# bcgsc/goldrush

Measured on AMD Instinct MI355X. Metric: reads/s through GoldRush-Path (hash + miBF query), higher is better.
Workload: dtype u64

## Files before the change

goldrush_amd/csrc/grp_kernels.inc:

```

__device__ inline uint64_t
window_lo(const uint32_t* sBases, uint32_t b)
{
  uint32_t bit = b * 2u;
  uint32_t wi = bit >> 5;
  uint32_t sh = bit & 31u;
  uint64_t lo = (uint64_t)sBases[wi] | ((uint64_t)sBases[wi + 1] << 32);
  uint64_t w = lo >> sh;
  if (sh) {
    w |= (uint64_t)sBases[wi + 2] << (64u - sh);
  }
  return w;
}

struct Win
{
  uint64_t lo;
  const uint32_t* src;
  uint32_t b;
};

__device__ inline Win
window_at(const uint32_t* sBases, uint32_t b)
{
// ... 749 lines not shown
      }
    }
    if (k == rank + 1) {
      stc(&f.ovf_ids[slot], id);
      return;
    }
    slot = (slot + 1) & f.ovf_mask;
  }
}

struct InsertTable
{
  unsigned long long* keys;
  unsigned long long* masks;
  unsigned long long* locs;
  uint32_t* slots;
  uint32_t* counter;
  uint64_t cap_mask;
};


struct DevStreamCtl
{
  uint32_t first = 0;
  uint32_t* tiles_done = nullptr;
  uint32_t* abort = nullptr;
  const uint32_t* abort_host = nullptr;
  grp_read_decision* dec = nullptr;
  uint32_t* next_tile = nullptr;
  uint32_t* park = nullptr;
  uint32_t n_tiles = 0;
  uint32_t early_park = 1;
  unsigned long long* executed = nullptr;
  grp_decide_params dp{};
  uint32_t* g_ids = nullptr;
  uint8_t* g_asg = nullptr;
  uint64_t* g_scratch = nullptr;
  uint32_t* ctl = nullptr;
  const uint32_t* cmd_host = nullptr;
  uint32_t* ack_host = nullptr;
  uint32_t n_reads = 0;
  uint32_t n_decidable = 0;
  uint32_t cmd_while_busy = 0;
  InsertTable tb{};
  unsigned long long timeout_ticks = 0;
  uint32_t* tile_ver = nullptr;
  uint32_t* fp_tab[2] = { nullptr, nullptr };
  uint32_t fp_mask = 0;
  uint32_t* rel = nullptr;
  uint32_t* dbg = nullptr;
  uint32_t n_fp = 0;
  uint32_t fp_off = 0;
  uint32_t fp_words = 0;
};

constexpr uint32_t STREAM_TILE_HELD = 0xFFFFFFFEu;
constexpr uint32_t STREAM_TILE_BUSY = 0xFFFFFFFDu;
constexpr uint32_t STREAM_REDO_NONE = 0xFFFFFFFFu;
constexpr uint32_t STREAM_FULL_RESET = 0x80000000u;

__device__ inline uint32_t
slot_fp(uint64_t b, uint32_t off)
{
  const uint32_t x = ((uint32_t)b ^ ((uint32_t)(b >> 32) * 0x85EBCA6Bu)) * 0x9E3779B1u + off;
  return x ? x : 1u;
}

constexpr unsigned long long IR_LOC_MASK = (1ull << 58) - 1ull;

__device__ inline uint32_t
fp_home(uint32_t fp, uint32_t mask)
{
  return (fp ^ (fp >> 15)) & mask;
}

__device__ inline void
fp_put(uint32_t* tab, uint32_t mask, uint32_t fp)
{
  uint32_t slot = fp_home(fp, mask);
  for (;;) {
    uint32_t cur = ldc(&tab[slot]);
    if (cur == 0u) {
      cur = atomicCAS(&tab[slot], 0u, fp);
      if (cur == 0u) {
        return;
      }
    }
    if (cur == fp) {
      return;
    }
    slot = (slot + 1u) & mask;
  }
}

__device__ inline bool
fp_has(const uint32_t* tab, uint32_t mask, uint32_t fp)
{
  uint32_t slot = fp_home(fp, mask);
  for (;;) {
    const uint32_t cur = tab[slot];
    if (cur == 0u) {
      return false;
    }
    if (cur == fp) {
      return true;
    }
// ... 1102 lines not shown
  uint32_t idx[H];
#pragma unroll
  for (int s = 0; s < H; ++s) {
    have[s] = look[s] && grp_claim_epoch(k[s]) == bv.epoch;
    idx[s] = grp_claim_record(k[s]);
  }
  uint32_t chain[H];
  unsigned long long rk[H], ro[H];
#pragma unroll
  for (int s = 0; s < H; ++s) {
    chain[s] = have[s] ? bv.rec_chain[idx[s]] : BATCH_NONE;
    rk[s] = have[s] ? bv.rec_key[idx[s]] : 0ull;
    ro[s] = have[s] ? bv.rec_old[idx[s]] : 0ull;
  }
#pragma unroll
  for (int s = 0; s < H; ++s) {
    if (have[s]) {
      if (chain[s] == BATCH_NONE) {
        const uint32_t j = (uint32_t)(rk[s] & ((1ull << 26) - 1ull)) >> 8;
        const uint32_t writer = bv.ins[(size_t)j * 6] - bv.first;
        d[s] = (writer >= reader && (ro[s] >> 63)) ? (uint32_t)ro[s] : d[s];
      } else {
        d[s] = batch_view_log(bv, rank[s] + 1, reader, d[s]);
      }
    }
  }
}

__device__ inline uint32_t
batch_view_log(const DevBatchView& bv, unsigned long long key, uint32_t reader, uint32_t cur)
{
  uint64_t slot = (key * 0x9E3779B97F4A7C15ULL) >> 18 & bv.log_mask;
  for (;;) {
    const unsigned long long k = bv.log_keys[slot];
    if (k == key) {
      break;
    }
    if (k == 0) {
      return cur;
    }
    slot = (slot + 1) & bv.log_mask;
  }
  uint32_t best_w = BATCH_NONE, best_old = cur;
  for (uint32_t e = bv.log_head[slot]; e != BATCH_NONE; e = bv.log_next[e]) {
    const uint32_t w = bv.log_writer[e];
    if (w >= reader && w <= best_w) {
      best_w = w;
      best_old = bv.log_old[e];
    }
  }
  return best_old;
}

template<int H, int FR, int WT, bool ST, bool VER = false, bool GT = false>
__global__ void __launch_bounds__(THREADS, (ST && H <= 3) ? 3 : ((!ST && H >= 4 && H <= 5) ? 3 : 1))
k_query(DevFilter f,
        DevReads rd,
        const DevSeeds* __restrict__ sd,
        uint32_t tile_len,
        uint64_t tile_begin,
        const uint32_t* __restrict__ tile_idx,
        uint32_t hist_cap,
        uint32_t distinct_limit,
        grp_tile_summary* __restrict__ tiles_out,
        grp_id_count* __restrict__ lists_out,
        uint64_t lists_cap,
        unsigned long long* __restrict__ ctr,
        uint32_t* __restrict__ flagged_out,
        uint32_t flagged_cap,
        uint32_t direct_stride,
        uint32_t blk0,
        DevStreamCtl sc,
        DevBatchView bv,
        uint32_t* __restrict__ gtab = nullptr)
{
  if constexpr (VER && !ST) {
    if (bv.redo_count != nullptr && blockIdx.x >= *bv.redo_count) {
      return;
    }
  }
  extern __shared__ uint4 smem4[];
  ulonglong2* sTab = reinterpret_cast<ulonglong2*>(smem4);
  const uint32_t hn = frame_seeds<H>(sd);
  uint32_t* sKeys;
  uint32_t* sCnts;
  uint32_t* sBases;
  if constexpr (GT) {
    sKeys = gtab + (size_t)blockIdx.x * (hist_cap + hist_cap / 2u);
    sCnts = sKeys + hist_cap;
    sBases = reinterpret_cast<uint32_t*>(sTab + hn * sd->wmax * 4u);
  } else {
    sKeys = reinterpret_cast<uint32_t*>(sTab + hn * sd->wmax * 4u);
    sCnts = sKeys + hist_cap;
    sBases = sCnts + hist_cap / 2u;
  }
  auto tab_word = [&](const uint32_t* p) -> uint32_t {
    if constexpr (GT) {
      return __hip_atomic_load(p, __ATOMIC_RELAXED, __HIP_MEMORY_SCOPE_AGENT);
    } else {
      return *p;
    }
  };
  __shared__ uint32_t sListN, sDistinct, sOverflow, sListOff, sListW;
  __shared__ uint32_t sRed[2 * (THREADS / 64)];
  __shared__ uint32_t sBest[2 * (THREADS / 64)];
  __shared__ uint32_t sTile;
  __shared__ unsigned long long sDirectWord;
  __shared__ uint32_t sInsWave[THREADS / 64 + 1];
  __shared__ uint32_t sEv, sAct;
  __shared__ uint32_t sHeldTile[2], sHeldPasses[2];
  __shared__ uint32_t sBuf;
  __shared__ uint32_t sCut;
  __shared__ uint32_t sOwnRedo[2], sOwnRedoN;
  __shared__ uint32_t sWalkEnd;
  __shared__ uint32_t sGen;

  load_tab(sTab, sd);
  uint32_t nxt = 0;
  uint32_t stop = 0;
  uint32_t my_ev = 0;
  uint32_t phase = 0;
  bool host_abort_seen = false;
  uint32_t ev_next = 0;
  uint32_t pending_event = 0;
  uint32_t* const sFp = (ST && sc.ctl && sc.n_fp) ? reinterpret_cast<uint32_t*>(reinterpret_cast<char*>(smem4) + sc.fp_off) : nullptr;
  if constexpr (ST) {
    if (threadIdx.x == 0) {
      sHeldTile[0] = sHeldTile[1] = STREAM_REDO_NONE;
      sHeldPasses[0] = sHeldPasses[1] = 0u;
      sBuf = 0u;
      sCut = 0u;
      sOwnRedoN = 0u;
      sWalkEnd = 0u;
      sGen = 1u;
      if (sc.dbg) {
        stc(&sc.dbg[blockIdx.x], 0x00000001u);
        stc(&sc.dbg[4095], gridDim.x);
        stc(&sc.dbg[4096 + (blockIdx.x & 1023u)], (uint32_t)wall_clock64());
        stc(&sc.dbg[5120 + (blockIdx.x & 1023u)], (__builtin_amdgcn_s_getreg((16 - 1) << 11 | 4) & 0xFFFFu) | (__builtin_amdgcn_s_getreg((4 - 1) << 11 | 20) << 16));
      }
      if (__hip_atomic_load(sc.abort_host, __ATOMIC_RELAXED, __HIP_MEMORY_SCOPE_SYSTEM)) {
        atomicMin(sc.park, 0u);
        atomicMax(sc.next_tile, STREAM_STOP);
        __hip_atomic_store(sc.abort, 1u, __ATOMIC_RELAXED, __HIP_MEMORY_SCOPE_AGENT);
        stop = 1u;
        host_abort_seen = true;
      }
      if (sc.ctl) {
        uint32_t ph0 = 0;
        if (!stream_register(sc, &my_ev, &ph0)) {
          stop = 1u;
          host_abort_seen = true;
        }
        sEv = ph0;
        sGen = ldc(sc.ctl + SCT_GEN);
        sWalkEnd = ldc(sc.ctl + SCT_SCAN_END) & ~STREAM_FULL_RESET;
        ev_next = my_ev;
      }
      nxt = atomicAdd(sc.next_tile, 1u);
    }
    if (sc.ctl) {
      __syncthreads();
      phase = sEv;
    }
  }
  for (;;) {
  uint32_t out_idx;
  if constexpr (ST) {
    if (__builtin_expect(pending_event != 0u, 0)) {
      pending_event = 0u;
      if (threadIdx.x == 0 && sc.dbg) {
        stc(&sc.dbg[blockIdx.x], 0x10000000u | (my_ev & 0xFFFFu));
        stc(&sc.dbg[1024 + (blockIdx.x & 1023u)], (uint32_t)wall_clock64());
      }
      if (threadIdx.x == 0) {
        sAct = host_abort_seen ? STREAM_ACT_EXIT : stream_idle(sc, &my_ev);
        sEv = my_ev;
        ev_next = my_ev;
      }
      __syncthreads();
      if (sAct == STREAM_ACT_EXIT) {
        return;
      }
      if (sAct == STREAM_ACT_INSERT) {
        if (sFp != nullptr && threadIdx.x < 2u) {
          const uint32_t th = sHeldTile[threadIdx.x];
          if (th != STREAM_REDO_NONE) {
            stc(&sc.tile_ver[th], STREAM_TILE_HELD);
          }
        }
        if (threadIdx.x == 0 && sc.dbg) {
          stc(&sc.dbg[blockIdx.x], 0x20000000u | (my_ev & 0xFFFFu));
        }
        StreamInsertDone done;
        if (!stream_apply_insert<H, WT>(f, rd, sd, sTab, sBases, sInsWave, &sAct, tile_len, sc, sEv, phase, ctr, lists_cap, tile_idx, done)) {
          return;
        }
        const bool keep_none = (done.scan_end & STREAM_FULL_RESET) != 0u;
        if (threadIdx.x == 0) {
          sWalkEnd = done.scan_end & ~STREAM_FULL_RESET;
          sGen = done.gen;
        }
        if (done.rank == 0u && threadIdx.x == 0) {
          atomicAdd(sc.executed + (keep_none ? EXE_INSERTS_KEPT_NONE : EXE_INSERTS_KEPT), 1ull);
        }
        {
          const uint32_t* const changed = sc.fp_tab[done.par];
          for (uint32_t hb = 0; hb < 2u; ++hb) {
            __syncthreads();
            const uint32_t th = sHeldTile[hb];
            if (sFp == nullptr || th == STREAM_REDO_NONE) {
              continue;
            }
            const uint32_t rh = rd.tile_read[tile_begin + th];
            const uint32_t rjh = rh - sc.first;
            if (rjh < done.resume_read) {
              __syncthreads();
              if (threadIdx.x == 0) {
                sHeldTile[hb] = STREAM_REDO_NONE;
              }
              continue;
            }
            bool dirty = keep_none;
            const uint32_t nfp = keep_none ? 0u : sHeldPasses[hb] * (uint32_t)THREADS * (uint32_t)H;
#pragma unroll 4
            for (uint32_t q = threadIdx.x; q < nfp; q += THREADS) {
              const uint32_t fp = sFp[hb * sc.fp_words + q];
              const bool hit = fp != 0u && fp_has(changed, sc.fp_mask, fp);
              dirty = dirty | hit;
            }
            const bool any_dirty = __syncthreads_or(dirty ? 1 : 0) != 0;
// ... 14 lines not shown
              sTile = (atomicAdd(&sc.tiles_done[rjh], 1u) + 1u == nt_h) ? 1u : 0u;
            }
            __syncthreads();
            if (sTile != 0u && threadIdx.x < 64u) {
              stream_decide(sc, rjh, rd.tile0[rh] - tile_begin, nt_h, tiles_out, lists_out, lists_cap, reinterpret_cast<uint32_t*>(sKeys), min(STREAM_LDS_TILES, hist_cap * 6u / 40u));
            }
          }
          __syncthreads();
          if (threadIdx.x == 0) {
            nxt = atomicAdd(sc.next_tile, 1u);
          }
          if (threadIdx.x == 0) {
            stop = 0u;
          }
        }
      }
      __syncthreads();
    }
    if (threadIdx.x == 0) {
      uint32_t pick = STREAM_STOP;
      bool from_dispenser = false;
      if (sc.ctl && ev_next != my_ev) {
      } else {
        if (sc.ctl && sOwnRedoN != 0u) {
          pick = sOwnRedo[--sOwnRedoN];
        }
        while (pick == STREAM_STOP && nxt < sc.n_tiles) {
          const uint32_t cand = tile_idx ? tile_idx[nxt] : nxt;
          if (sc.ctl && nxt < sWalkEnd) {
            const uint32_t v = ldc(&sc.tile_ver[cand]);
            if (v == STREAM_TILE_HELD || v == STREAM_TILE_BUSY || (v != 0u && v == sGen)) {
              nxt = atomicAdd(sc.next_tile, 1u);
              continue;
            }
            if (v != 0u) {
              atomicAdd(sc.executed + EXE_REDONE_LOST, 1ull);
            }
          }
          pick = cand;
          from_dispenser = true;
        }
        if (stop && from_dispenser) {
          const uint32_t rj = rd.tile_read[tile_begin + pick] - sc.first;
          if (rj >= __hip_atomic_load(sc.park, __ATOMIC_RELAXED, __HIP_MEMORY_SCOPE_AGENT)) {
            pick = STREAM_STOP;
            from_dispenser = false;
          }
        }
      }
      sTile = pick;
      if (from_dispenser) {
        nxt = atomicAdd(sc.next_tile, 1u);
      }
      if (pick != STREAM_STOP && sc.ctl != nullptr && blockIdx.x < 32u) {
        stream_relay(sc);
      } else if (pick != STREAM_STOP && blockIdx.x < 32u) {
        if (__hip_atomic_load(sc.abort_host, __ATOMIC_RELAXED, __HIP_MEMORY_SCOPE_SYSTEM)) {
          atomicMin(sc.park, 0u);
          atomicMax(sc.next_tile, STREAM_STOP);
          __hip_atomic_store(sc.abort, 1u, __ATOMIC_RELAXED, __HIP_MEMORY_SCOPE_AGENT);
        }
      }
    }
    if (threadIdx.x == 0 && sc.dbg) {
      stc(&sc.dbg[blockIdx.x], 0x30000000u | (sTile & 0x0FFFFFFFu));
    }
    __syncthreads();
    out_idx = sTile;
    if (out_idx == STREAM_STOP) {
      if (!sc.ctl) {
        return;
      }
      pending_event = 1u;
      continue;
    }
  } else {
    out_idx = tile_idx ? tile_idx[blockIdx.x] : blockIdx.x + blk0;
  }
  const uint64_t t = tile_begin + out_idx;
  const uint32_t r = rd.tile_read[t];
  const uint32_t ti = (uint32_t)(t - rd.tile0[r]);
  if constexpr (VER && !ST) {
    if (bv.skip_read_ins != nullptr && r - bv.first < bv.skip_reads) {
      const uint32_t ji = bv.skip_read_ins[r - bv.first];
      if (ji != 0xFFFFFFFFu && ti >= bv.ins[(size_t)ji * 6 + 1] && ti < bv.ins[(size_t)ji * 6 + 2]) {
        return;
      }
    }
  }
  const uint32_t len = rd.len[r];
  const gr::geom::TileExtent ext = tile_extent(sd, tile_len, len, ti);
  const uint32_t start = ext.start, Lp = ext.Lp, frames = ext.frames;

  const uint32_t boff = stage_bases(sBases, rd.packed, rd.word_off[r], len, start, Lp);
  for (uint32_t i = threadIdx.x; i < hist_cap; i += THREADS) {
    sKeys[i] = 0u;
    if (i < hist_cap / 2u) {
      sCnts[i] = 0u;
    }
  }
  if (threadIdx.x == 0) {
    sListN = 0;
    sListW = 0;
    sDistinct = 0;
    sOverflow = 0;
    if constexpr (ST) {
      sCut = 0u;
      if (sFp != nullptr) {
        if (sc.n_fp > 1u) {
          sBuf ^= 1u;
        }
        sHeldTile[sBuf] = STREAM_REDO_NONE;
      }
    }
  }
  __syncthreads();
  if constexpr (ST) {
    if (threadIdx.x == 0) {
      atomicAdd(sc.executed + EXE_PROBES, (unsigned long long)frames * hn);
    }
  }
  uint32_t* const fp_cur = (ST && sFp != nullptr) ? sFp + sBuf * sc.fp_words : nullptr;

  uint32_t n_hit = 0, n_miss = 0;
  uint32_t last[H];
#pragma unroll
  for (int s = 0; s < H; ++s) {
    last[s] = Lp - sd->span[s];
  }
  const QuadLane ql = quad_lane();
  constexpr bool ROT = quad_rotated<H, FR, WT, ST, VER, GT>();
  const uint32_t pbytes = quad_piece_bytes(ql.sub);

  const uint32_t n_left = (H >= 2 && H <= GRP_H_GROUP && WT != GRP_WT_LONG) ? sd->n_left : 0u;
  constexpr uint32_t OV = (uint32_t)H - 1u, USE = 64u - OV;
  static_assert(THREADS == 256, "the helper-lane layout below is written for four waves per workgroup (my_wave == 3 is the last one, FBH = 3 * USE + 64)");
  constexpr uint32_t FBH = gr::geom::helper_pass_frames(H);
  const uint32_t ftile = frames_per_tile(sd, tile_len);
  const bool helper = n_left != 0u && (ftile + FBH * FR - 1u) / (FBH * FR) == (ftile + THREADS * FR - 1u) / (THREADS * FR);
  const uint32_t FB = helper ? FBH : (uint32_t)THREADS;
  const uint32_t my_wave = threadIdx.x >> 6, my_lane = threadIdx.x & 63u;
  const uint32_t my_off = helper ? (my_wave * USE + my_lane) : threadIdx.x;
  const bool my_real = helper ? (my_wave == 3u || my_lane < USE) : true;
  const bool my_tail_wave = helper ? my_wave == 3u : true;
  const uint32_t passes = (frames + FB * FR - 1u) / (FB * FR);
  uint64_t bk[FR][H];
  uint32_t off[FR][H];
  bool live_j[FR];
  auto positions = [&](uint32_t pp, uint64_t (&bk_)[FR][H], uint32_t (&off_)[FR][H], bool (&lv)[FR]) {
  if (n_left != 0u) {
#pragma unroll
    for (int j = 0; j < FR; ++j) {
      const uint32_t fr_raw = (pp * FR + j) * FB + my_off;
      const uint32_t fr = min(fr_raw, frames - 1u);
      lv[j] = my_real && fr_raw < frames;
      uint64_t hL, hRL, hR, hRR;
      seed_halves<WT, true, true>(sTab, sd, n_left, window_at(sBases, boff + fr), hL, hRL, hR, hRR);
      const uint64_t hv0 = (hL ^ hR) + (hRL ^ hRR);
#pragma unroll
      for (int s = 0; s < H; ++s) {
        uint64_t hv = hv0;
        if (s != 0) {
          uint64_t nR = __shfl_down((unsigned long long)hR, (unsigned)s, 64);
          uint64_t nRR = __shfl_down((unsigned long long)hRR, (unsigned)s, 64);
          if (my_tail_wave && my_lane + (uint32_t)s >= 64u) {
            uint64_t a, b;
            seed_halves<WT, false, true>(sTab, sd, n_left, window_at(sBases, boff + min(fr_raw + (uint32_t)s, frames - 1u)), a, b, nR, nRR);
          }
          if (lv[j]) {
            if (fr <= last[s]) {
              hv = (srol_small(hL, (uint32_t)s) ^ nR) + (hRL ^ srol_small(nRR, (uint32_t)s));
            } else {
              hv = seed_hash_t<WT>(sTab, sd, s, window_at(sBases, boff + last[s]));
            }
          }
        }
        const Probe p = grp_locate(f, hv);
        bk_[j][s] = p.b;
        off_[j][s] = p.off;
        if constexpr (ST) {
          if (fp_cur != nullptr) {
            fp_cur[((pp * FR + (uint32_t)j) * (uint32_t)THREADS + threadIdx.x) * (uint32_t)H + (uint32_t)s] = lv[j] ? slot_fp(p.b, p.off) : 0u;
          }
        }
      }
    }
  } else {
#pragma unroll
    for (int j = 0; j < FR; ++j) {
      const uint32_t fr_raw = (pp * FR + j) * THREADS + threadIdx.x;
      const uint32_t fr = min(fr_raw, frames - 1u);
      lv[j] = fr_raw < frames;
#pragma unroll
      for (int s = 0; s < H; ++s) {
        if (!seed_on<H>(s, frame_seeds<H>(sd))) {
          bk_[j][s] = 0;
          off_[j][s] = 0;
          if constexpr (ST) {
            if (fp_cur != nullptr) {
              fp_cur[((pp * FR + (uint32_t)j) * (uint32_t)THREADS + threadIdx.x) * (uint32_t)H + (uint32_t)s] = 0u;
            }
          }
          continue;
        }
        const uint64_t hv = seed_hash_t<WT>(sTab, sd, s, window_at(sBases, boff + min(fr, last[s])));
        const Probe p = grp_locate(f, hv);
        bk_[j][s] = p.b;
        off_[j][s] = p.off;
        if constexpr (ST) {
          if (fp_cur != nullptr) {
            fp_cur[((pp * FR + (uint32_t)j) * (uint32_t)THREADS + threadIdx.x) * (uint32_t)H + (uint32_t)s] = lv[j] ? slot_fp(p.b, p.off) : 0u;
          }
        }
      }
    }
  }
  };
  constexpr bool PIPE = (ST || FR == 1) && H <= GRP_H_GROUP;
  if constexpr (PIPE) {
    if (passes > 0u) {
      positions(0u, bk, off, live_j);
    }
  }
  for (uint32_t pass = 0; pass < passes; ++pass) {
    if constexpr (ST) {
      if (sc.ctl && sFp == nullptr && pass != 0u && __hip_atomic_load(sc.abort, __ATOMIC_RELAXED, __HIP_MEMORY_SCOPE_WORKGROUP) != 0u) {
        if (r - sc.first >= ldc(sc.park)) {
          if ((threadIdx.x & 63u) == 0u) {
            sCut = 1u;
          }
          break;
        }
      }
    }
    if constexpr (H <= GRP_H_GROUP) {
      uint4 piece[FR][H][4];
      if constexpr (!PIPE) {
        positions(pass, bk, off, live_j);
      }
#pragma unroll
      for (int j = 0; j < FR; ++j) {
#pragma unroll
        for (int s = 0; s < H; ++s) {
          piece[j][s][0] = quad_read<ROT, 0>(f.buckets, bk[j][s], ql, pbytes);
          piece[j][s][1] = quad_read<ROT, 1>(f.buckets, bk[j][s], ql, pbytes);
          piece[j][s][2] = quad_read<ROT, 2>(f.buckets, bk[j][s], ql, pbytes);
          piece[j][s][3] = quad_read<ROT, 3>(f.buckets, bk[j][s], ql, pbytes);
        }
      }
      uint64_t bk_next[PIPE ? FR : 1][PIPE ? H : 1];
      uint32_t off_next[PIPE ? FR : 1][PIPE ? H : 1];
      bool live_next[PIPE ? FR : 1];
      if constexpr (PIPE) {
        if (pass + 1u < passes) {
          positions(pass + 1u, bk_next, off_next, live_next);
        }
      }
#pragma unroll
      for (int j = 0; j < FR; ++j) {
        const bool live = live_j[j];
        bool all = live;
        uint32_t idv[H];
        uint64_t vrank[VER ? H : 1], vbl[VER ? H : 1];
        bool vneed[VER ? H : 1], vamb[VER ? H : 1];
#pragma unroll
        for (int s = 0; s < H; ++s) {
          const QuadAnswer mine = quad_result<ROT>(piece[j][s], off[j][s], ql);
          all = all && mine.bit;
          uint32_t d = mine.id;

          if (mine.lr >= GRP_BUCKET_IDS && live) {
            d = grp_ovf_get(f, f.super[bk[j][s] >> GRP_SUPER_SHIFT] + mine.rel + mine.lr);
          }
          if constexpr (VER) {
            const uint32_t fl = bv.floor[r - bv.floor_first];
            const uint32_t floor_id = fl & 0x7FFFFFFFu;
            vrank[s] = f.super[bk[j][s] >> GRP_SUPER_SHIFT] + mine.rel + mine.lr;
            vbl[s] = bk[j][s] * 64ull + mine.lr;
            vneed[s] = live && mine.bit && (d & 0x7FFFFFFFu) >= floor_id;
            vamb[s] = (fl >> 31) != 0u && (d & 0x7FFFFFFFu) == floor_id;
          }
          idv[s] = d;
        }
        if (!all) {
          continue;
        }
        if constexpr (VER) {
          batch_view_multi<H>(bv, vrank, vbl, vneed, vamb, r - bv.first, idv);
        }
        uint32_t ids[H];
#pragma unroll
        for (int s = 0; s < H; ++s) {
          const uint32_t d = idv[s];
          const uint32_t id = (d > 0x80000000u) ? (d & 0x7FFFFFFFu) : d;
          if (id == 0u) {
            ++n_miss;
          } else {
            ++n_hit;
          }
          bool dup = false;
#pragma unroll
          for (int u = 0; u < s; ++u) {
            dup = dup || (ids[u] == id);
          }
          ids[s] = id;
          if (id != 0u && !dup) {
            hist_add16(sKeys, sCnts, hist_cap, id, &sDistinct, distinct_limit, &sOverflow);
          }
        }
      }
      if constexpr (PIPE) {
        if (pass + 1u < passes) {
#pragma unroll
          for (int j = 0; j < FR; ++j) {
            live_j[j] = live_next[j];
#pragma unroll
            for (int s = 0; s < H; ++s) {
              bk[j][s] = bk_next[j][s];
              off[j][s] = off_next[j][s];
            }
          }
        }
      }
    } else {
      static_assert(FR == 1 && !PIPE, "the many-seed form runs one frame per lane and pass");
      constexpr int NG = (H + GRP_H_GROUP - 1) / GRP_H_GROUP;
      positions(pass, bk, off, live_j);
      const bool live = live_j[0];
      bool all = live;
      uint32_t idv[H];
      uint64_t vrank[VER ? H : 1], vbl[VER ? H : 1];
      bool vneed[VER ? H : 1], vamb[VER ? H : 1];
#pragma unroll
      for (int s = 0; s < H; ++s) {
        idv[s] = 0u;
        if constexpr (VER) {
          vrank[s] = 0;
          vbl[s] = 0;
          vneed[s] = false;
          vamb[s] = false;
        }
      }
#pragma unroll
      for (int gi = 0; gi < NG; ++gi) {
        uint4 piece[GRP_H_GROUP][4];
#pragma unroll
        for (int q = 0; q < GRP_H_GROUP; ++q) {
          const int s = gi * GRP_H_GROUP + q;
          if (seed_on<H>(s, hn)) {
            piece[q][0] = quad_read<ROT, 0>(f.buckets, bk[0][s], ql, pbytes);
            piece[q][1] = quad_read<ROT, 1>(f.buckets, bk[0][s], ql, pbytes);
            piece[q][2] = quad_read<ROT, 2>(f.buckets, bk[0][s], ql, pbytes);
            piece[q][3] = quad_read<ROT, 3>(f.buckets, bk[0][s], ql, pbytes);
          }
        }
#pragma unroll
        for (int q = 0; q < GRP_H_GROUP; ++q) {
          const int s = gi * GRP_H_GROUP + q;
          if (!seed_on<H>(s, hn)) {
            continue;
          }
          const QuadAnswer mine = quad_result<ROT>(piece[q], off[0][s], ql);
          all = all && mine.bit;
          uint32_t d = mine.id;
          if (mine.lr >= GRP_BUCKET_IDS && live) {
            d = grp_ovf_get(f, f.super[bk[0][s] >> GRP_SUPER_SHIFT] + mine.rel + mine.lr);
          }
          if constexpr (VER) {
            const uint32_t fl = bv.floor[r - bv.floor_first];
            const uint32_t floor_id = fl & 0x7FFFFFFFu;
            vrank[s] = f.super[bk[0][s] >> GRP_SUPER_SHIFT] + mine.rel + mine.lr;
            vbl[s] = bk[0][s] * 64ull + mine.lr;
            vneed[s] = live && mine.bit && (d & 0x7FFFFFFFu) >= floor_id;
            vamb[s] = (fl >> 31) != 0u && (d & 0x7FFFFFFFu) == floor_id;
          }
          idv[s] = d;
        }
      }
      if (all) {
        if constexpr (VER) {
// ... 579 lines not shown
```

goldrush_amd/csrc/grp_query.inc:

```

namespace {

constexpr uint32_t GT_SLICE = 256;

struct QueryGeom
{
  uint32_t hist_cap;
  uint32_t distinct_limit;
  size_t lds;
  bool global_table = false;
};

QueryGeom
query_geom(const grp_ctx* c, bool full)
{
  const uint32_t h = c->params.h, tile = c->params.tile;
  const uint64_t max_ids = (uint64_t)tile_frames(c) * h;
  auto lds_of = [&](uint32_t cap) { return tab_bytes(c) + (size_t)cap * 6 + bases_bytes(tile + c->params.k + h); };
  const uint32_t cap_full = (uint32_t)((max_ids + (uint64_t)THREADS * h + 2 + 1023) / 1024 * 1024);
  const uint32_t forced_small = c->sw.small_hist;
  QueryGeom g;
  g.hist_cap = cap_full;
  if (!full) {
    if (forced_small && forced_small < cap_full && forced_small > (uint32_t)THREADS * h + 64) {
// ... 114 lines not shown
      if (e == hipSuccess) {
        return GRP_OK;
      }
      (void)hipGetLastError();
      return set_err(c, GRP_ERR_BUSY, "cooperative launch of a resumable window refused: %s", hipGetErrorString(e));
    }
    a.launch(kern, (uint32_t)q.n_launch, launch_lds, c->stream);
    return GRP_OK;
  };
  constexpr int SFR = (HH <= 3) ? 2 : 1;
  if (g.global_table) {
    if (q.stream_ctl || q.direct_stride) {
      return set_err(c, GRP_ERR_STATE, "launch_query: a global count table in a streaming / zero-copy launch");
    }
    const uint64_t words = (uint64_t)g.hist_cap + g.hist_cap / 2u;
    if (const int rc = ensure_dev(c, c->d_gtab, words * GT_SLICE); rc != GRP_OK) {
      return rc;
    }
    const bool ver = c->view && !q.plain;
    QueryArgs a = query_args(c, r, q);
    for (uint64_t off = 0; off < q.n_launch; off += GT_SLICE) {
      const uint32_t nb = (uint32_t)std::min<uint64_t>(GT_SLICE, q.n_launch - off);
      a.idx = q.d_tile_idx ? q.d_tile_idx + off : nullptr;
      a.blk0 = q.d_tile_idx ? q.blk0 : q.blk0 + (uint32_t)off;
      if (ver) {
        if (a.bv.redo_count && off) {
          break;
        }
        auto kern = k_query<HH, 1, QWT, false, true, true>;
        if (const int rc = ensure_lds(c, kern, g.lds); rc != GRP_OK) {
          return rc;
        }
        a.launch(kern, nb, g.lds, c->stream);
      } else {
        auto kern = k_query<HH, 1, QWT, false, false, true>;
        if (const int rc = ensure_lds(c, kern, g.lds); rc != GRP_OK) {
          return rc;
        }
        a.launch(kern, nb, g.lds, c->stream);
      }
    }
    return GRP_OK;
  }
  if (c->view && !q.stream_ctl && !q.plain) {
    return go(k_query<HH, SFR, QWT, false, true>);
  }
  if (q.stream_ctl) {
    auto kern = k_query<HH, 1, QWT, true>;
    int per_cu = 0;
    HIP_TRY(c, hipOccupancyMaxActiveBlocksPerMultiprocessor(&per_cu, kern, THREADS, g.lds));
    DevStreamCtl sc_fit = *q.stream_ctl;
    QueryGeom g_fit = g;
    sc_fit.n_fp = 0;
    if (q.stream_ctl->ctl && q.stream_ctl->n_fp) {
      const int keep_env = c->sw.stream_keep;
      const uint32_t fb = gr::geom::helper_pass_frames(HH);
      const uint32_t passes = (tile_frames(c) + fb - 1u) / fb;
      const uint32_t words = passes * (uint32_t)THREADS * (uint32_t)HH;
      const int want_cu = std::min(per_cu, 3);
      for (int nf = std::min<int>(keep_env, (int)q.stream_ctl->n_fp); nf >= 1; --nf) {
        const size_t lds = g.lds + (size_t)nf * words * 4u;
        int fit = 0;
        if (lds <= LDS_PER_WORKGROUP && ensure_lds(c, kern, lds) == GRP_OK && hipOccupancyMaxActiveBlocksPerMultiprocessor(&fit, kern, THREADS, lds) == hipSuccess && fit >= want_cu) {
          sc_fit.n_fp = (uint32_t)nf;
          sc_fit.fp_off = (uint32_t)g.lds;
          sc_fit.fp_words = words;
          g_fit.lds = lds;
          break;
        }
        (void)hipGetLastError();
      }
    }
    q.stream_ctl = &sc_fit;
    launch_lds = g_fit.lds;
    int rc = ensure_lds(c, kern, launch_lds);
    if (rc != GRP_OK) {
      return rc;
    }
    const int cap_per_cu = c->sw.stream_wgs_per_cu;
    per_cu = std::min(per_cu, cap_per_cu > 0 ? cap_per_cu : 3);
    const uint64_t resident = std::min<uint64_t>((uint64_t)std::max(per_cu, 1) * (uint64_t)std::max(c->n_cus, 1), STREAM_REL_WGS);
    q.n_launch = std::min<uint64_t>(q.n_launch, resident);
    c->dbg_stream_lds = (uint32_t)launch_lds;
    c->dbg_stream_grid = (uint32_t)q.n_launch;
    return go(kern);
  }
  return go(k_query<HH, SFR, QWT, false>);
}

int
launch_query(grp_ctx* c, const grp_reads* r, const QueryLaunch& q)
{
  int rc = GRP_OK;
  DISPATCH_H_SPAN(c, (rc = launch_query_wt<HH, WW>(c, r, q)));
  return rc;
}

struct QueryRun
{
  uint64_t t0 = 0, nt = 0, probes = 0;
  uint64_t used = 0;
  uint64_t flagged = 0;
};

int
slot_query_bufs(grp_ctx* c, QuerySlot& sl, uint64_t nt, uint64_t lists)
{
  HIP_TRY(c, sl.d_tiles.ensure(nt));
  HIP_TRY(c, sl.d_lists.ensure(lists));
  HIP_TRY(c, sl.d_flag_idx.ensure(nt));
  return GRP_OK;
}

int
slot_dec_scratch(grp_ctx* c, QuerySlot& sl, uint64_t nt)
{
  if (nt + 1 > sl.d_dec_cap) {
    clear_all(sl.d_dec_ids, sl.d_dec_asg, sl.d_dec_scratch);
    sl.d_dec_cap = 0;
    const uint64_t cap = nt + nt / 4 + 64;
    HIP_TRY(c, sl.d_dec_ids.reset(cap));
    HIP_TRY(c, sl.d_dec_asg.reset(cap));
    HIP_TRY(c, sl.d_dec_scratch.reset(cap));
// ... 265 lines not shown
```

goldrush_amd/csrc/grpath_hip.hip:

```cpp
#include "grp_buffers.h"
#include "grp_device.h"
#include "grp_stream_proto.h"
#include "host/gr_stream_stripes.hpp"
#include "host/gr_tile_geom.hpp"
#include "host/gr_tiles_core.hpp"
#include "host/gr_bam.hpp"
#include "host/gr_gather_word.hpp"

#include "../../include/grpath.h"
#include "../../include/grpath_ingest.h"

#include <algorithm>
#include <cstdarg>
#include <cstdio>
#include <cstring>
#include <chrono>
#include <cmath>
#include <mutex>
#include <string>
#include <thread>
#include <vector>


namespace {
// ... 97 lines not shown
  uint32_t first_read = 0;
};

constexpr int FQ_TEXT_SLOTS = 3;

struct CtxStreams
{
  hipStream_t stream = nullptr;
  hipStream_t stream2 = nullptr;
  hipStream_t stream3 = nullptr;
  ~CtxStreams()
  {
    for (hipStream_t s : { stream3, stream2, stream }) {
      if (s) {
        (void)hipStreamDestroy(s);
      }
    }
  }
};

struct grp_ctx : CtxStreams
{
  int device = 0;
  std::string arch;
  bool coherent_arch = false;
  BatchRun batch;
  grp_params params{};
  std::vector<std::string> seeds;
  DevSeeds h_seeds{};
  DevBuf<DevSeeds> d_seeds;
  DevBuf<uint32_t> d_gtab;
  DevFilter f{};
  DevBuf<uint32_t> bv;
  DevBuf<uint4> buckets;
  DevBuf<ulonglong2> far;
  DevBuf<unsigned long long> ovf_keys;
  DevBuf<uint32_t> ovf_ids;
  uint64_t nsb = 0;
  uint64_t n_bv_words = 0;
  uint64_t n_ovf = 0;
  uint64_t n_far = 0;
  uint32_t uniform_weight = 0;

  struct Switches
  {
    bool no_direct = false;
    bool stream_resume_off = false;
    bool no_early_park = false;
    int trace_abort = 0;
    uint32_t small_hist = 0;
    uint32_t batch_epochs = GRP_EPOCH_MAX;
    int stream_keep = 2;
    int stream_wgs_per_cu = 0;
    bool stream_debug = false;
    double stream_wait_s = 2.0;
    bool verify_strict = false;
    long batch_ovf_cap = 0;
    uint32_t batch_overlap_shift = 59;
    bool batch_verify_off = false;
    bool shared_halves_off = false;
    bool debug_stats = false;
  } sw;
  struct OverlapBuf
  {
    DevBuf<unsigned long long> d_samples;
    DevBuf<uint32_t> d_n;
    DevBuf<unsigned long long> d_tab;
    DevBuf<uint32_t> d_prev;
  } ovl;
  uint64_t n_overlap_calls = 0;
  uint64_t n_batch_sweeps = 0;
  uint64_t n_stream_keep[8] = { 0, 0, 0, 0, 0, 0, 0, 0 };
  uint64_t n_stream_idle_exits = 0, n_stream_coop_refused = 0;
  uint64_t n_flagged_tiles = 0, n_flagged_distinct = 0, n_flagged_list = 0;
  uint64_t n_verify_impossible = 0;
  uint64_t n_verify_tiles = 0, n_verify_queried = 0, n_verify_flagged = 0, n_verify_fallbacks = 0, n_verify_uncertified = 0, n_verify_unpatched = 0;
  uint64_t n_direct_windows = 0, n_direct_fallbacks = 0, n_general_windows = 0, n_redo_launches = 0;
  uint64_t n_chunks = 0;
  DevBuf<uint64_t> d_super;
  struct Prealloc
  {
    double occupancy = 0.0;
    bool started = false;
    std::thread worker;
    DevBuf<uint4> units;
    uint64_t units_buckets = 0;
    DevBuf<ulonglong2> far;
  } pre;
  double finalize_times[6] = { 0, 0, 0, 0, 0, 0 };
  bool finalized = false;
  int n_cus = 0;
  std::mutex fill_mutex;
  DevBuf<uint32_t> d_ntc;
  uint32_t ntc_sbits = 0;
  DevBuf<uint2> d_ntc_chunks;
  DevBuf<uint32_t> d_ntc_extra;
  QuerySlot slot[2];
  QuerySlot* q = &slot[0];
  struct Carry
  {
    bool valid = false;
    uint32_t slot = 0;
    const grp_reads* reads = nullptr;
    uint32_t first = 0, count = 0;
    uint64_t tile_off = 0;
  } carry;
// ... 364 lines not shown
  HIP_TRY(c, sl.d_dec_raw.reset(cap + 2));
  HIP_TRY(c, sl.h_dec_raw.reset(cap + 2, hipHostMallocDefault));
  memset(sl.h_dec_raw, 0, 2 * sizeof(grp_read_decision));
  sl.d_dec = sl.d_dec_raw + 2;
  sl.h_dec = sl.h_dec_raw + 2;
  sl.h_qctr = reinterpret_cast<uint64_t*>(sl.h_dec_raw.p);
  return GRP_OK;
}

template<typename T>
int
ensure_dev(grp_ctx* c, DevBuf<T>& b, uint64_t want)
{
  HIP_TRY(c, b.ensure(want));
  return GRP_OK;
}

constexpr size_t LDS_PER_WORKGROUP = 160 * 1024 - 512;
static_assert(GRP_DEV_MAX_H * GRP_DEV_MAX_W * 4u * sizeof(ulonglong2) + bases_bytes(GRP_MAX_TILE + GRP_MAX_SPAN + GRP_DEV_MAX_H) <= LDS_PER_WORKGROUP,
              "a tile of the longest span does not fit the LDS beside the seed tables");
}

#include "grp_query.inc"

namespace {

grp_ctx::Switches
read_switches()
{
  grp_ctx::Switches s;
  const auto set = [](const char* name) { return getenv(name) != nullptr; };
  const auto off = [](const char* name) {
    const char* e = getenv(name);
    return e && !strcmp(e, "off");
  };
  s.no_direct = set("GRP_NO_DIRECT");
  s.stream_resume_off = off("GRP_STREAM_RESUME");
  s.no_early_park = set("GRP_NO_EARLY_PARK");
  if (const char* e = getenv("GRP_TRACE_ABORT")) {
    s.trace_abort = e[0] == '2' ? 2 : 1;
  }
  if (const char* e = getenv("GRP_SMALL_HIST")) {
    s.small_hist = (uint32_t)atoi(e) / 2u * 2u;
  }
  if (const char* e = getenv("GRP_BATCH_EPOCHS")) {
    s.batch_epochs = (uint32_t)std::min<long>(std::max<long>(atol(e), 1), (long)GRP_EPOCH_MAX);
  }
  if (const char* e = getenv("GRP_STREAM_KEEP")) {
    s.stream_keep = std::max(0, std::min(2, atoi(e)));
  }
  if (const char* e = getenv("GRP_STREAM_WGS_PER_CU")) {
    s.stream_wgs_per_cu = atoi(e);
  }
  s.stream_debug = set("GRP_STREAM_DEBUG");
  if (const char* e = getenv("GRP_STREAM_WAIT_S")) {
    s.stream_wait_s = atof(e);
  }
  s.verify_strict = set("GRP_VERIFY_STRICT");
  if (const char* e = getenv("GRP_BATCH_OVF_CAP")) {
    s.batch_ovf_cap = atol(e);
  }
  if (const char* e = getenv("GRP_BATCH_OVERLAP_SHIFT")) {
    s.batch_overlap_shift = (uint32_t)std::min(63, std::max(52, atoi(e)));
  }
  s.batch_verify_off = off("GRP_BATCH_VERIFY");
  s.shared_halves_off = off("GRP_SHARED_HALVES");
  s.debug_stats = set("GRP_DEBUG_STATS");
  return s;
}

int
build_seed_tables(grp_ctx* c)
{
  DevSeeds& sd = c->h_seeds;
  memset(&sd, 0, sizeof(sd));
  sd.h = c->params.h;
  sd.k = c->params.k;
  sd.wmax = 0;
  const size_t sp0 = c->seeds[0].size();
  if (sp0 == 0 || (sp0 != c->params.k && sp0 + 1 != c->params.k)) {
    return set_err(c, GRP_ERR_INVALID, "seed 0 has span %zu, expected k = %u or k-1 = %u", sp0, c->params.k, c->params.k - 1);
  }
  for (uint32_t s = 0; s < sd.h; ++s) {
    const std::string& p = c->seeds[s];
    if (p.size() != sp0 + s) {
      return set_err(c, GRP_ERR_INVALID, "seed %u has span %zu, expected k+%u = %u or k-1+%u = %u", s, p.size(), s, c->params.k + s, s, c->params.k - 1 + s);
    }
    sd.span[s] = (uint32_t)p.size();
    uint32_t w = 0;
    for (uint32_t q = 0; q < p.size(); ++q) {
      if (p[q] == '1') {
        if (w >= GRP_DEV_MAX_W) {
          return set_err(c, GRP_ERR_INVALID, "seed weight > %d unsupported", GRP_DEV_MAX_W);
        }
        sd.shift[s][w] = 2u * q;
        for (uint32_t b = 0; b < 4; ++b) {
          sd.tab[s][w][b].x = srol_n(BASE_SEED[b], sd.span[s] - 1u - q);
          sd.tab[s][w][b].y = srol_n(BASE_SEED[3u - b], q);
        }
        ++w;
      } else if (p[q] != '0') {
        return set_err(c, GRP_ERR_INVALID, "seed %u contains '%c'", s, p[q]);
      }
    }
    sd.weight[s] = w;
    sd.wmax = std::max(sd.wmax, w);
// ... 1408 lines not shown
```

Before: 479,400.

## Prefetch next stream tile's read metadata and bases during final passes

In the streaming query kernel, each wave uses its last passes of the current tile to fetch the next dispensed tile's read index, length, word offset and packed bases into a second LDS buffer. It also computes the first-pass hash positions for that next tile. When the next tile matches the prefetched one, the dependent global-load chain (tile_read, tile0, len, word_off, packed) and the first positions call are skipped. This costs extra LDS, registers and a more complex pass loop, and it may lower occupancy or fingerprint-buffer capacity. The host checks that the added LDS still fits before enabling it.

```diff
diff --git a/goldrush_amd/csrc/grp_kernels.inc b/goldrush_amd/csrc/grp_kernels.inc
--- a/goldrush_amd/csrc/grp_kernels.inc
+++ b/goldrush_amd/csrc/grp_kernels.inc
@@ -825,6 +825,7 @@
   uint32_t n_fp = 0;
   uint32_t fp_off = 0;
   uint32_t fp_words = 0;
+  uint32_t ahead_off = 0;
 };
 
 constexpr uint32_t STREAM_TILE_HELD = 0xFFFFFFFEu;
@@ -2033,6 +2034,29 @@
   return best_old;
 }
 
+template<int H>
+struct TileHash
+{
+  const uint32_t* bases;
+  uint32_t boff, frames;
+  uint32_t last[H];
+};
+
+constexpr uint32_t AH_HAVE = 0;
+constexpr uint32_t AH_CAND = 1;
+constexpr uint32_t AH_READ = 2;
+constexpr uint32_t AH_TI = 3;
+constexpr uint32_t AH_LEN = 4;
+constexpr uint32_t AH_WOFF = 5;
+constexpr uint32_t AH_DONE = 7;
+constexpr uint32_t AH_WORDS = 8;
+
+__device__ __forceinline__ uint32_t
+ah_uniform(uint32_t v)
+{
+  return __builtin_amdgcn_readfirstlane(v);
+}
+
 template<int H, int FR, int WT, bool ST, bool VER = false, bool GT = false>
 __global__ void __launch_bounds__(THREADS, (ST && H <= 3) ? 3 : ((!ST && H >= 4 && H <= 5) ? 3 : 1))
 k_query(DevFilter f,
@@ -2095,6 +2119,14 @@
   __shared__ uint32_t sOwnRedo[2], sOwnRedoN;
   __shared__ uint32_t sWalkEnd;
   __shared__ uint32_t sGen;
+  constexpr bool AHEAD = ST && H <= GRP_H_GROUP;
+  __shared__ uint32_t sAhPos;
+  __shared__ uint32_t sAhWave[AHEAD ? (THREADS / 64) * AH_WORDS : 1];
+  __shared__ uint32_t sAhHit[4];
+  uint32_t* const sBases2 = (AHEAD && sc.ahead_off) ? reinterpret_cast<uint32_t*>(reinterpret_cast<char*>(smem4) + sc.ahead_off) : nullptr;
+  uint64_t bk[FR][H];
+  uint32_t off[FR][H];
+  bool live_j[FR];
 
   load_tab(sTab, sd);
   uint32_t nxt = 0;
@@ -2114,6 +2146,13 @@
       sOwnRedoN = 0u;
       sWalkEnd = 0u;
       sGen = 1u;
+      sAhPos = STREAM_REDO_NONE;
+      if constexpr (AHEAD) {
+        for (uint32_t w = 0; w < (uint32_t)THREADS / 64u; ++w) {
+          sAhWave[w * AH_WORDS + AH_HAVE] = 0u;
+          sAhWave[w * AH_WORDS + AH_DONE] = STREAM_REDO_NONE;
+        }
+      }
       if (sc.dbg) {
         stc(&sc.dbg[blockIdx.x], 0x00000001u);
         stc(&sc.dbg[4095], gridDim.x);
@@ -2158,6 +2197,11 @@
         sAct = host_abort_seen ? STREAM_ACT_EXIT : stream_idle(sc, &my_ev);
         sEv = my_ev;
         ev_next = my_ev;
+        if constexpr (AHEAD) {
+          for (uint32_t w = 0; w < (uint32_t)THREADS / 64u; ++w) {
+            sAhWave[w * AH_WORDS + AH_DONE] = STREAM_REDO_NONE;
+          }
+        }
       }
       __syncthreads();
       if (sAct == STREAM_ACT_EXIT) {
@@ -2278,6 +2322,19 @@
       if (from_dispenser) {
         nxt = atomicAdd(sc.next_tile, 1u);
       }
+      if constexpr (AHEAD) {
+        bool hit = pick != STREAM_STOP && sBases2 != nullptr;
+        for (uint32_t w = 0; w < (uint32_t)THREADS / 64u; ++w) {
+          hit = hit && sAhWave[w * AH_WORDS + AH_DONE] == pick;
+          sAhWave[w * AH_WORDS + AH_DONE] = STREAM_REDO_NONE;
+          sAhWave[w * AH_WORDS + AH_HAVE] = 0u;
+        }
+        sAhHit[0] = hit ? 1u : 0u;
+        sAhHit[1] = sAhWave[AH_READ];
+        sAhHit[2] = sAhWave[AH_TI];
+        sAhHit[3] = sAhWave[AH_LEN];
+        sAhPos = STREAM_REDO_NONE;
+      }
       if (pick != STREAM_STOP && sc.ctl != nullptr && blockIdx.x < 32u) {
         stream_relay(sc);
       } else if (pick != STREAM_STOP && blockIdx.x < 32u) {
@@ -2304,8 +2361,12 @@
     out_idx = tile_idx ? tile_idx[blockIdx.x] : blockIdx.x + blk0;
   }
   const uint64_t t = tile_begin + out_idx;
-  const uint32_t r = rd.tile_read[t];
-  const uint32_t ti = (uint32_t)(t - rd.tile0[r]);
+  bool ahead_hit = false;
+  if constexpr (AHEAD) {
+    ahead_hit = ah_uniform(sAhHit[0]) != 0u;
+  }
+  const uint32_t r = ahead_hit ? ah_uniform(sAhHit[1]) : rd.tile_read[t];
+  const uint32_t ti = ahead_hit ? ah_uniform(sAhHit[2]) : (uint32_t)(t - rd.tile0[r]);
   if constexpr (VER && !ST) {
     if (bv.skip_read_ins != nullptr && r - bv.first < bv.skip_reads) {
       const uint32_t ji = bv.skip_read_ins[r - bv.first];
@@ -2314,11 +2375,20 @@
       }
     }
   }
-  const uint32_t len = rd.len[r];
+  const uint32_t len = ahead_hit ? ah_uniform(sAhHit[3]) : rd.len[r];
   const gr::geom::TileExtent ext = tile_extent(sd, tile_len, len, ti);
   const uint32_t start = ext.start, Lp = ext.Lp, frames = ext.frames;
 
-  const uint32_t boff = stage_bases(sBases, rd.packed, rd.word_off[r], len, start, Lp);
+  uint32_t boff;
+  if (ahead_hit) {
+    const uint32_t nw = ((start + Lp + 15u) >> 4) - (start >> 4) + 4u;
+    for (uint32_t i = threadIdx.x; i < nw; i += blockDim.x) {
+      sBases[i] = sBases2[i];
+    }
+    boff = start & 15u;
+  } else {
+    boff = stage_bases(sBases, rd.packed, rd.word_off[r], len, start, Lp);
+  }
   for (uint32_t i = threadIdx.x; i < hist_cap; i += THREADS) {
     sKeys[i] = 0u;
     if (i < hist_cap / 2u) {
@@ -2332,6 +2402,11 @@
     sOverflow = 0;
     if constexpr (ST) {
       sCut = 0u;
+      if constexpr (AHEAD) {
+        if (sBases2 != nullptr && frames <= 3u * (uint32_t)THREADS * (uint32_t)FR) {
+          sAhPos = nxt < sc.n_tiles ? nxt : STREAM_REDO_NONE;
+        }
+      }
       if (sFp != nullptr) {
         if (sc.n_fp > 1u) {
           sBuf ^= 1u;
@@ -2349,10 +2424,13 @@
   uint32_t* const fp_cur = (ST && sFp != nullptr) ? sFp + sBuf * sc.fp_words : nullptr;
 
   uint32_t n_hit = 0, n_miss = 0;
-  uint32_t last[H];
+  TileHash<H> th_cur;
+  th_cur.bases = sBases;
+  th_cur.boff = boff;
+  th_cur.frames = frames;
 #pragma unroll
   for (int s = 0; s < H; ++s) {
-    last[s] = Lp - sd->span[s];
+    th_cur.last[s] = Lp - sd->span[s];
   }
   const QuadLane ql = quad_lane();
   constexpr bool ROT = quad_rotated<H, FR, WT, ST, VER, GT>();
@@ -2370,10 +2448,10 @@
   const bool my_real = helper ? (my_wave == 3u || my_lane < USE) : true;
   const bool my_tail_wave = helper ? my_wave == 3u : true;
   const uint32_t passes = (frames + FB * FR - 1u) / (FB * FR);
-  uint64_t bk[FR][H];
-  uint32_t off[FR][H];
-  bool live_j[FR];
-  auto positions = [&](uint32_t pp, uint64_t (&bk_)[FR][H], uint32_t (&off_)[FR][H], bool (&lv)[FR]) {
+  auto positions = [&](const TileHash<H>& th, uint32_t pp, uint32_t* fp_dst, uint64_t (&bk_)[FR][H], uint32_t (&off_)[FR][H], bool (&lv)[FR]) {
+  const uint32_t* const sBases = th.bases;
+  const uint32_t boff = th.boff, frames = th.frames;
+  const uint32_t (&last)[H] = th.last;
   if (n_left != 0u) {
 #pragma unroll
     for (int j = 0; j < FR; ++j) {
@@ -2405,8 +2483,8 @@
         bk_[j][s] = p.b;
         off_[j][s] = p.off;
         if constexpr (ST) {
-          if (fp_cur != nullptr) {
-            fp_cur[((pp * FR + (uint32_t)j) * (uint32_t)THREADS + threadIdx.x) * (uint32_t)H + (uint32_t)s] = lv[j] ? slot_fp(p.b, p.off) : 0u;
+          if (fp_dst != nullptr) {
+            fp_dst[((pp * FR + (uint32_t)j) * (uint32_t)THREADS + threadIdx.x) * (uint32_t)H + (uint32_t)s] = lv[j] ? slot_fp(p.b, p.off) : 0u;
           }
         }
       }
@@ -2423,8 +2501,8 @@
           bk_[j][s] = 0;
           off_[j][s] = 0;
           if constexpr (ST) {
-            if (fp_cur != nullptr) {
-              fp_cur[((pp * FR + (uint32_t)j) * (uint32_t)THREADS + threadIdx.x) * (uint32_t)H + (uint32_t)s] = 0u;
+            if (fp_dst != nullptr) {
+              fp_dst[((pp * FR + (uint32_t)j) * (uint32_t)THREADS + threadIdx.x) * (uint32_t)H + (uint32_t)s] = 0u;
             }
           }
           continue;
@@ -2434,8 +2512,8 @@
         bk_[j][s] = p.b;
         off_[j][s] = p.off;
         if constexpr (ST) {
-          if (fp_cur != nullptr) {
-            fp_cur[((pp * FR + (uint32_t)j) * (uint32_t)THREADS + threadIdx.x) * (uint32_t)H + (uint32_t)s] = lv[j] ? slot_fp(p.b, p.off) : 0u;
+          if (fp_dst != nullptr) {
+            fp_dst[((pp * FR + (uint32_t)j) * (uint32_t)THREADS + threadIdx.x) * (uint32_t)H + (uint32_t)s] = lv[j] ? slot_fp(p.b, p.off) : 0u;
           }
         }
       }
@@ -2445,9 +2523,24 @@
   constexpr bool PIPE = (ST || FR == 1) && H <= GRP_H_GROUP;
   if constexpr (PIPE) {
     if (passes > 0u) {
-      positions(0u, bk, off, live_j);
-    }
-  }
+      if (!ahead_hit) {
+        positions(th_cur, 0u, fp_cur, bk, off, live_j);
+      } else {
+#pragma unroll
+        for (int j = 0; j < FR; ++j) {
+          live_j[j] = my_real && (uint32_t)j * FB + my_off < frames;
+          if (fp_cur != nullptr) {
+#pragma unroll
+            for (int s = 0; s < H; ++s) {
+              fp_cur[((uint32_t)j * (uint32_t)THREADS + threadIdx.x) * (uint32_t)H + (uint32_t)s] = live_j[j] ? slot_fp(bk[j][s], off[j][s]) : 0u;
+            }
+          }
+        }
+      }
+    }
+  }
+  const bool ahead_on = AHEAD && sBases2 != nullptr;
+  uint32_t* const ah = AHEAD ? sAhWave + ah_uniform(my_wave) * AH_WORDS : nullptr;
   for (uint32_t pass = 0; pass < passes; ++pass) {
     if constexpr (ST) {
       if (sc.ctl && sFp == nullptr && pass != 0u && __hip_atomic_load(sc.abort, __ATOMIC_RELAXED, __HIP_MEMORY_SCOPE_WORKGROUP) != 0u) {
@@ -2462,7 +2555,66 @@
     if constexpr (H <= GRP_H_GROUP) {
       uint4 piece[FR][H][4];
       if constexpr (!PIPE) {
-        positions(pass, bk, off, live_j);
+        positions(th_cur, pass, fp_cur, bk, off, live_j);
+      }
+      uint32_t ah_step = 0;
+      uint32_t ah0 = 0, ah1 = 0, ah2 = 0, ah3 = 0;
+      if constexpr (AHEAD) {
+        const uint32_t left = passes - 1u - pass;
+        if (ahead_on && left <= 2u) {
+          uint32_t have = ah_uniform(ah[AH_HAVE]);
+          const uint32_t target = 3u - left;
+          if (have == 0u) {
+            const uint32_t pos = ah_uniform(sAhPos);
+            if (pos != STREAM_REDO_NONE) {
+              const uint32_t cand = tile_idx ? tile_idx[pos] : pos;
+              if (my_lane == 0u) {
+                ah[AH_CAND] = cand;
+              }
+              ah0 = rd.tile_read[tile_begin + cand];
+              if (target >= 2u) {
+                if (my_lane == 0u) {
+                  ah[AH_READ] = ah0;
+                }
+                have = 1u;
+              } else {
+                ah_step = 1u;
+              }
+            }
+          }
+          if (have == 1u && ah_step == 0u) {
+            const uint32_t rn = ah_uniform(ah[AH_READ]);
+            ah0 = reinterpret_cast<const uint32_t*>(rd.tile0 + rn)[0];
+            ah1 = rd.len[rn];
+            const uint64_t wo = rd.word_off[rn];
+            ah2 = (uint32_t)wo;
+            ah3 = (uint32_t)(wo >> 32);
+            if (target >= 3u) {
+              if (my_lane == 0u) {
+                ah[AH_TI] = (uint32_t)tile_begin + ah[AH_CAND] - ah0;
+                ah[AH_LEN] = ah1;
+                ah[AH_WOFF] = ah2;
+                ah[AH_WOFF + 1u] = ah3;
+              }
+              have = 2u;
+            } else {
+              ah_step = 2u;
+            }
+          }
+          if (have == 2u && ah_step == 0u && left == 0u) {
+            const uint32_t len_n = ah_uniform(ah[AH_LEN]);
+            const gr::geom::TileExtent en = tile_extent(sd, tile_len, len_n, ah_uniform(ah[AH_TI]));
+            const uint32_t w0 = en.start >> 4, w_read = (len_n + 15u) >> 4;
+            const uint32_t nw = ((en.start + en.Lp + 15u) >> 4) - w0 + 4u;
+            if (en.frames != 0u && nw <= 128u) {
+              const uint64_t wo = (uint64_t)ah_uniform(ah[AH_WOFF]) | ((uint64_t)ah_uniform(ah[AH_WOFF + 1u]) << 32);
+              const uint32_t wa = w0 + my_lane, wb = wa + 64u;
+              ah0 = (my_lane < nw && wa < w_read) ? rd.packed[wo + wa] : 0u;
+              ah1 = (my_lane + 64u < nw && wb < w_read) ? rd.packed[wo + wb] : 0u;
+              ah_step = 3u;
+            }
+          }
+        }
       }
 #pragma unroll
       for (int j = 0; j < FR; ++j) {
@@ -2477,9 +2629,55 @@
       uint64_t bk_next[PIPE ? FR : 1][PIPE ? H : 1];
       uint32_t off_next[PIPE ? FR : 1][PIPE ? H : 1];
       bool live_next[PIPE ? FR : 1];
-      if constexpr (PIPE) {
+      bool have_next = pass + 1u < passes;
+      if constexpr (AHEAD) {
+        if (ahead_on && pass == 0u && passes > 3u && threadIdx.x == 0) {
+          sAhPos = nxt < sc.n_tiles ? nxt : STREAM_REDO_NONE;
+        }
+        uint32_t pp = pass + 1u;
+        uint32_t* fp_dst = fp_cur;
+        if (ah_step == 1u) {
+          if (my_lane == 0u) {
+            ah[AH_READ] = ah0;
+            ah[AH_HAVE] = 1u;
+          }
+        } else if (ah_step == 2u) {
+          if (my_lane == 0u) {
+            ah[AH_TI] = (uint32_t)tile_begin + ah[AH_CAND] - ah0;
+            ah[AH_LEN] = ah1;
+            ah[AH_WOFF] = ah2;
+            ah[AH_WOFF + 1u] = ah3;
+            ah[AH_HAVE] = 2u;
+          }
+        } else if (ah_step == 3u) {
+          const gr::geom::TileExtent en = tile_extent(sd, tile_len, ah_uniform(ah[AH_LEN]), ah_uniform(ah[AH_TI]));
+          const uint32_t nw = ((en.start + en.Lp + 15u) >> 4) - (en.start >> 4) + 4u;
+          if (my_lane < nw) {
+            sBases2[my_lane] = ah0;
+          }
+          if (my_lane + 64u < nw) {
+            sBases2[my_lane + 64u] = ah1;
+          }
+          th_cur.bases = sBases2;
+          th_cur.boff = en.start & 15u;
+          th_cur.frames = en.frames;
+#pragma unroll
+          for (int s = 0; s < H; ++s) {
+            th_cur.last[s] = en.Lp - sd->span[s];
+          }
+          pp = 0u;
+          fp_dst = nullptr;
+          have_next = true;
+          if (my_lane == 0u) {
+            ah[AH_DONE] = ah[AH_CAND];
+          }
+        }
+        if (have_next) {
+          positions(th_cur, pp, fp_dst, bk_next, off_next, live_next);
+        }
+      } else if constexpr (PIPE) {
         if (pass + 1u < passes) {
-          positions(pass + 1u, bk_next, off_next, live_next);
+          positions(th_cur, pass + 1u, fp_cur, bk_next, off_next, live_next);
         }
       }
 #pragma unroll
@@ -2536,7 +2734,7 @@
         }
       }
       if constexpr (PIPE) {
-        if (pass + 1u < passes) {
+        if (have_next) {
 #pragma unroll
           for (int j = 0; j < FR; ++j) {
             live_j[j] = live_next[j];
@@ -2551,7 +2749,7 @@
     } else {
       static_assert(FR == 1 && !PIPE, "the many-seed form runs one frame per lane and pass");
       constexpr int NG = (H + GRP_H_GROUP - 1) / GRP_H_GROUP;
-      positions(pass, bk, off, live_j);
+      positions(th_cur, pass, fp_cur, bk, off, live_j);
       const bool live = live_j[0];
       bool all = live;
       uint32_t idv[H];
diff --git a/goldrush_amd/csrc/grp_query.inc b/goldrush_amd/csrc/grp_query.inc
--- a/goldrush_amd/csrc/grp_query.inc
+++ b/goldrush_amd/csrc/grp_query.inc
@@ -190,23 +190,39 @@
     DevStreamCtl sc_fit = *q.stream_ctl;
     QueryGeom g_fit = g;
     sc_fit.n_fp = 0;
+    sc_fit.ahead_off = 0;
+    if (HH <= GRP_H_GROUP && !c->sw.stream_ahead_off) {
+      const size_t lds = g.lds + bases_bytes(c->params.tile + c->params.k + c->params.h);
+      int fit = 0;
+      if (lds <= LDS_PER_WORKGROUP && ensure_lds(c, kern, lds) == GRP_OK && hipOccupancyMaxActiveBlocksPerMultiprocessor(&fit, kern, THREADS, lds) == hipSuccess && fit >= std::min(per_cu, 3)) {
+        sc_fit.ahead_off = (uint32_t)g.lds;        g_fit.lds = lds;
+      } else {
+        (void)hipGetLastError();
+      }
+    }
+    const size_t lds_fp0 = g_fit.lds;
     if (q.stream_ctl->ctl && q.stream_ctl->n_fp) {
       const int keep_env = c->sw.stream_keep;
       const uint32_t fb = gr::geom::helper_pass_frames(HH);
       const uint32_t passes = (tile_frames(c) + fb - 1u) / fb;
       const uint32_t words = passes * (uint32_t)THREADS * (uint32_t)HH;
       const int want_cu = std::min(per_cu, 3);
-      for (int nf = std::min<int>(keep_env, (int)q.stream_ctl->n_fp); nf >= 1; --nf) {
-        const size_t lds = g.lds + (size_t)nf * words * 4u;
-        int fit = 0;
-        if (lds <= LDS_PER_WORKGROUP && ensure_lds(c, kern, lds) == GRP_OK && hipOccupancyMaxActiveBlocksPerMultiprocessor(&fit, kern, THREADS, lds) == hipSuccess && fit >= want_cu) {
-          sc_fit.n_fp = (uint32_t)nf;
-          sc_fit.fp_off = (uint32_t)g.lds;
-          sc_fit.fp_words = words;
-          g_fit.lds = lds;
-          break;
-        }
-        (void)hipGetLastError();
+      for (int nf = std::min<int>(keep_env, (int)q.stream_ctl->n_fp); nf >= 1 && sc_fit.n_fp == 0u; --nf) {
+        for (const size_t base : { lds_fp0, g.lds }) {
+          const size_t lds = base + (size_t)nf * words * 4u;
+          int fit = 0;
+          if (lds <= LDS_PER_WORKGROUP && ensure_lds(c, kern, lds) == GRP_OK && hipOccupancyMaxActiveBlocksPerMultiprocessor(&fit, kern, THREADS, lds) == hipSuccess && fit >= want_cu) {
+            sc_fit.n_fp = (uint32_t)nf;
+            sc_fit.fp_off = (uint32_t)base;
+            sc_fit.fp_words = words;
+            if (base == g.lds) {
+              sc_fit.ahead_off = 0;
+            }
+            g_fit.lds = lds;
+            break;
+          }
+          (void)hipGetLastError();
+        }
       }
     }
     q.stream_ctl = &sc_fit;
diff --git a/goldrush_amd/csrc/grpath_hip.hip b/goldrush_amd/csrc/grpath_hip.hip
--- a/goldrush_amd/csrc/grpath_hip.hip
+++ b/goldrush_amd/csrc/grpath_hip.hip
@@ -173,6 +173,7 @@
     uint32_t batch_epochs = GRP_EPOCH_MAX;
     int stream_keep = 2;
     int stream_wgs_per_cu = 0;
+    bool stream_ahead_off = false;
     bool stream_debug = false;
     double stream_wait_s = 2.0;
     bool verify_strict = false;
@@ -643,6 +644,7 @@
   if (const char* e = getenv("GRP_STREAM_WGS_PER_CU")) {
     s.stream_wgs_per_cu = atoi(e);
   }
+  s.stream_ahead_off = off("GRP_STREAM_AHEAD");
   s.stream_debug = set("GRP_STREAM_DEBUG");
   if (const char* e = getenv("GRP_STREAM_WAIT_S")) {
     s.stream_wait_s = atof(e);
```

Result: no change. 477,700 (-0.4%).
